# CODEJIN/multi_speaker_tts

Hardware: AMD Instinct MI355X
Metric: mel-frames/sec (train step) at batch 32x(128 tok,800 mel) (higher is better)
Workload: dtype f32

## Files before the change

include/mstts.h:

```cpp
#ifndef MSTTS_H_
#define MSTTS_H_
#include <stdint.h>
#ifdef __cplusplus
extern "C" {
#endif

typedef void* mstts_stream_t;

enum { MSTTS_OK = 0, MSTTS_ERR_SHAPE = -1, MSTTS_ERR_DTYPE = -2, MSTTS_ERR_ALIGN = -3, MSTTS_ERR_LAUNCH = -4 };
enum { MSTTS_ACT_NONE = 0, MSTTS_ACT_RELU = 1, MSTTS_ACT_TANH = 2, MSTTS_ACT_SIGMOID = 3 };

const char* mstts_last_error(void);
int mstts_abi_version(void);
int mstts_debug_park_cus(int32_t n_workgroups, int64_t microseconds, uint32_t* done_count, mstts_stream_t s);

typedef struct {
    const float* A; const float* B; float* C; const float* bias;
    int64_t M, N, K;
    int64_t lda, ldb, ldc;
    int32_t trans_a, trans_b;
    int32_t win_T, win_C, win_pad;
    int32_t act, accumulate, split_k;
    int64_t batch, stride_a, stride_b, stride_c;
    float alpha;
    int32_t win_dil;
} mstts_gemm_desc;
int mstts_gemm_f32(const mstts_gemm_desc* d, mstts_stream_t s);
int mstts_gemm_tail_split(int32_t on);
int mstts_gemm_split3(int32_t on);
int mstts_gemm_split_big(int32_t on);
int mstts_gemm_big_min_workgroups(int32_t f32_split, int32_t bf16);
int mstts_gemm_deterministic(int32_t on);
int mstts_gemm_bf16(const mstts_gemm_desc* d, mstts_stream_t s);
int mstts_gemm_bf16_autocut(int32_t on);
int mstts_gemm_bf16_big(int32_t on);

int mstts_philox_keep_mask(uint8_t* out, int64_t n, uint64_t seed, uint32_t stream_id, float keep_prob, mstts_stream_t s);
int mstts_philox_keep_mask_rows(uint8_t* out, int64_t outer, int64_t B, int64_t inner, uint64_t seed, uint32_t stream_id,
                                uint64_t sample0, float keep_prob, mstts_stream_t s);

int mstts_embedding_fwd(const int32_t* token, const float* table, float* out, int64_t n, int64_t vocab, int64_t width, mstts_stream_t s);
int mstts_embedding_bwd(const int32_t* token, const float* dout, float* dtable, int64_t n, int64_t vocab, int64_t width, mstts_stream_t s);

int mstts_bn_train_fwd(const float* x, const float* gamma, const float* beta, float* moving_mean, float* moving_var,
                       float* y, float* save_mean, float* save_rstd, const uint8_t* keep_mask, float keep_prob,
                       float momentum, float eps, int64_t rows, int64_t C, float* ws, mstts_stream_t s);
int mstts_bn_infer_fwd(const float* x, const float* gamma, const float* beta, const float* moving_mean,
                       const float* moving_var, float* y, float eps, int64_t rows, int64_t C, mstts_stream_t s);
int mstts_bn_train_bwd(const float* dy, const float* x, const float* gamma, const float* save_mean, const float* save_rstd,
                       const uint8_t* keep_mask, float keep_prob, int32_t act, float* dz, float* dgamma, float* dbeta,
                       float* dbias, int64_t rows, int64_t C, float* ws, mstts_stream_t s);

int mstts_dropout(const float* x, const uint8_t* keep_mask, float keep_prob, float* y, int64_t n, mstts_stream_t s);
int mstts_relu_dropout_bwd(const float* dy, const float* y_saved, const uint8_t* keep_mask, float keep_prob, float* dx, int64_t n, mstts_stream_t s);
int mstts_colsum(const float* x, int64_t rows, int64_t C, int64_t ld, float* out, int32_t accumulate, mstts_stream_t s);
// ... 399 lines not shown
```

multi_speaker_tts_amd/csrc/gemm.hip:

```cpp
#include "gemm_tile.h"
#include <type_traits>
#include <cmath>
#include <cstdlib>

namespace mstts {

constexpr int BK = 32;
constexpr int BN = 128;

struct GemmArgs : GemmTileArgs {
    int body, tail_s, tail_kps;
    int band;
};

template <int R, bool VEC>
struct LoaderKC {
    static constexpr int NV = R * BK / 4 / 256;
    float4 reg[NV];
    const float* ubase;
    unsigned voff[NV], rmask;
    int t_row[NV], tap, kc, ld_;
    __device__ __forceinline__ void prepare(const float* __restrict__ base, long ld, int row0, int k0, int rows,
                                            int wT, int wC, int wpad, int wdil) {
        const int k4 = threadIdx.x & 7, r = threadIdx.x >> 3;
        rmask = 0; ld_ = (int)ld;
#pragma unroll
        for (int i = 0; i < NV; ++i) {
            const int row = row0 + r + i * 32;
            if (row < rows) rmask |= 1u << i;
            voff[i] = (unsigned)((r + i * 32) * (int)ld) + (wT > 0 ? 0u : (unsigned)(k4 * 4));
            if (wT > 0) t_row[i] = row % wT;
        }
        if (wT > 0) {
            const int k = k0 + k4 * 4;
            tap = k / wC; kc = k - tap * wC;
// ... 223 lines not shown
#include "gemm_split.inc"

}

using namespace mstts;

static int g_tail_split = 1;
extern "C" int mstts_gemm_tail_split(int32_t on) { g_tail_split = on != 0; return MSTTS_OK; }
static int g_split3 = 1;
extern "C" int mstts_gemm_split3(int32_t on) { g_split3 = on != 0; return MSTTS_OK; }
static int g_split_big = 1;
extern "C" int mstts_gemm_split_big(int32_t on) { g_split_big = on != 0; return MSTTS_OK; }
static int g_split_big_min = 160;
namespace mstts { void gemm_bf16_set_big_min(int n); }
extern "C" int mstts_gemm_big_min_workgroups(int32_t f32_split, int32_t bf16) {
    if (f32_split > 0) g_split_big_min = f32_split;
    gemm_bf16_set_big_min(bf16);
    return MSTTS_OK;
}
static thread_local int t_deterministic = 0;
extern "C" int mstts_gemm_deterministic(int32_t on) { t_deterministic = on != 0; return MSTTS_OK; }
namespace mstts { int gemm_deterministic_now() { return t_deterministic; } }

extern "C" int mstts_gemm_f32(const mstts_gemm_desc* d, mstts_stream_t stream) {
    GemmArgs g;
    bool vec;
    const int rc = gemm_args_from(d, "gemm", BK, 1 << 24, &g, &vec);
    if (rc != MSTTS_OK || g.M == 0 || g.N == 0) return rc;
    const int batch = d->batch > 0 ? (int)d->batch : 1, split = g.split_k, kps = g.k_per_split;
    const bool skinny = d->M <= 32;
    int bm = skinny ? 32 : 128, tail_s = 1, tail_rem = 0;
    const bool split3 = g_split3 && !skinny && d->K >= 160 && (d->win_T <= 0 || (d->win_T >= BK && d->win_C >= BK)) && gemm_ready<GemmSplit>();
    if (!skinny) {
        const double t128 = (double)cdiv(d->M, 128) * cdiv(d->N, BN) * batch * split, t64 = (double)cdiv(d->M, 64) * cdiv(d->N, BN) * batch * split;
        const double e128 = t128 / (ceil(t128 / 256.0) * 256.0), e64 = t64 / (ceil(t64 / 256.0) * 256.0);
        if (e64 * 0.95 > e128 && !split3) bm = 64;
        if (g_tail_split && !t_deterministic && batch == 1 && split == 1 && (d->act == MSTTS_ACT_NONE || !d->accumulate)) {
            double best = (bm == 128 ? ceil(t128 / 256.0) : ceil(t64 / 256.0) * 0.54);
            const int ktiles = cdiv(d->K, BK);
            for (int cand = 128; cand >= (split3 ? 128 : 64); cand -= 64) {
                const long t = (long)cdiv(d->M, cand) * cdiv(d->N, BN);
                int rem = (int)(t % 256);
                if (d->act != MSTTS_ACT_NONE) rem = (int)(t - (t - rem) / cdiv(d->N, BN) * cdiv(d->N, BN));
                if (split3 && t <= 128) rem = (int)t;
                else if (t <= 256 || rem == 0 || rem > 128) continue;
                int s = 256 / rem;
                if (s > 16) s = 16;
                if (s > ktiles / 8) s = ktiles / 8;
                if (s < 2) continue;
                const double c = ((double)(t / 256) + 1.25 / s + 0.06) * (cand == 128 ? 1.0 : 0.54);
                if (c < best) { best = c; bm = cand; tail_s = s; tail_rem = rem; }
            }
        }
    }
    hipStream_t st = (hipStream_t)stream;
    const bool ta = d->trans_a != 0, tb = d->trans_b != 0, win = g.win_T > 0;
    {
        const long big_wgs = (long)cdiv(d->M, GSB_BM) * cdiv(d->N, GSB_BN) * batch * split;
        if (split3 && g_split_big && d->M >= 192 && d->N >= 192 && big_wgs >= g_split_big_min && d->lda < (1 << 22) && d->ldb < (1 << 22) &&
            (d->win_T <= 0 || (d->win_T >= GSB_BK && d->win_C >= GSB_BK)) && (d->act == MSTTS_ACT_NONE || split == 1) && gemm_ready<GemmSplitBig>()) {
            const int kpsb = gemm_k_per_split(g.K, split, GSB_BK);
            g.k_per_split = kpsb;
            g.body = 0; g.tail_s = 1; g.tail_kps = kpsb; g.band = 0;
            dim3 gridb(cdiv(d->M, GSB_BM) * cdiv(d->N, GSB_BN), 1, batch * split);
            gemm_launch<GemmSplitBig>(g, ta, tb, vec, win, gridb, st);
            MSTTS_CHECK_LAUNCH("gemm_f32 (split, 256 x 256 tile)");
            return MSTTS_OK;
        }
    }
    const int tiles = cdiv(d->M, bm) * cdiv(d->N, BN);
    g.body = tiles; g.tail_s = 1; g.tail_kps = kps;
    g.band = (split3 && tail_s == 1 && cdiv(d->N, BN) > 8) ? 8 : 0;
    if (tail_s > 1) {
        const int rem = tail_rem, tiles_n = cdiv(d->N, BN);
        g.body = tiles - rem; g.tail_s = tail_s;
        g.tail_kps = (cdiv(g.K, BK) + tail_s - 1) / tail_s * BK;
        if (!d->accumulate) {
            const long r0 = (long)(g.body / tiles_n) * bm;
            if (hipMemset2DAsync(d->C + r0 * d->ldc, (size_t)d->ldc * 4, 0, (size_t)d->N * 4, (size_t)(d->M - r0), st) != hipSuccess)
                MSTTS_REQUIRE(false, MSTTS_ERR_LAUNCH, "gemm: clearing the tail tiles failed");
        }
    }
    dim3 grid(g.body + (tiles - g.body) * g.tail_s, 1, batch * split);
    if (split3) gemm_launch<GemmSplit>(g, ta, tb, vec, win, grid, st);
    else if (skinny) gemm_launch<GemmF32<32>>(g, ta, tb, vec, win, grid, st);
    else if (bm == 64) gemm_launch<GemmF32<64>>(g, ta, tb, vec, win, grid, st);
    else gemm_launch<GemmF32<128>>(g, ta, tb, vec, win, grid, st);
    MSTTS_CHECK_LAUNCH("gemm_f32");
    if (tail_s > 1 && d->act != MSTTS_ACT_NONE) {
        const long r0 = (long)(g.body / cdiv(d->N, BN)) * bm;
        const long n = (d->M - r0) * d->N;
        hipLaunchKernelGGL(gemm_tail_act_kernel, dim3((unsigned)cdiv(n, 256)), dim3(256), 0, st, d->C + r0 * d->ldc, d->ldc, (int)d->N, n, d->act);
        MSTTS_CHECK_LAUNCH("gemm_f32 tail activation");
    }
    return MSTTS_OK;
}
```

multi_speaker_tts_amd/csrc/gemm_split.inc:

```

typedef __bf16 gs_bf16x8 __attribute__((ext_vector_type(8)));
typedef __bf16 gs_bf16x4 __attribute__((ext_vector_type(4)));
constexpr int GS_BM = 128, GS_LD = 40;
constexpr int GS_PLANE = 128 * GS_LD;

struct Split3 { gs_bf16x4 hi, mid, lo; };
__device__ __forceinline__ uint32_t gs_cvt_pk(float a, float b) {
    uint32_t r;
    asm("v_cvt_pk_bf16_f32 %0, %1, %2" : "=v"(r) : "v"(a), "v"(b));
    return r;
}
__device__ __forceinline__ float gs_sub(float a, uint32_t b_bits) {
    float r;
    asm("v_sub_f32 %0, %1, %2" : "=v"(r) : "v"(a), "v"(b_bits));
    return r;
}
__device__ __forceinline__ void gs_split2(float x0, float x1, uint32_t& hi, uint32_t& mid, uint32_t& lo) {
    hi = gs_cvt_pk(x0, x1);
    x0 = gs_sub(x0, hi << 16); x1 = gs_sub(x1, hi & 0xffff0000u);
    mid = gs_cvt_pk(x0, x1);
    x0 = gs_sub(x0, mid << 16); x1 = gs_sub(x1, mid & 0xffff0000u);
    lo = gs_cvt_pk(x0, x1);
}
__device__ __forceinline__ Split3 gs_split4(float a, float b, float c, float d) {
// ... 227 lines not shown
                acc[i][j] = __builtin_amdgcn_mfma_f32_32x32x16_bf16(f[i], fb[j][pb], acc[i][j], 0, 0, 0);
    };

    if (nt > 0) {
        load(kbeg);
        store(0);
        load(kbeg + GSB_BK);
        gemm_barrier();
        for (int t = 0; t < nt; ++t) {
            const __bf16* buf = gs_lds + (t & 1) * GSB_BUF;
            ldB(buf); ldA(fa0, buf, 0); ldA(fa1, buf, 1);
            mm(fa0, 0); mm(fa0, 1); mm(fa0, 2);
            ldA(fa0, buf, 2);
            store((t + 1) & 1);
            load(kbeg + (t + 2) * GSB_BK);
            mm(fa1, 0); mm(fa1, 1);
            mm(fa0, 0);
            gemm_barrier();
        }
    }
    gemm_store_tile<4, 2>(g, acc, C, m0 + wrow, n0 + wcol, lane, split == 0, g.split_k > 1);
}

struct GemmSplit {
    using Args = GemmArgs;
    static constexpr int THREADS = GS_THREADS;
    static constexpr size_t LDS_BYTES = GS_LDS_BYTES;
    template <bool TA, bool TB, bool VEC, bool WIN> static constexpr auto kernel() { return &gemm_split_kernel<TA, TB, VEC, WIN>; }
};
struct GemmSplitBig {
    using Args = GemmArgs;
    static constexpr int THREADS = GSB_THREADS;
    static constexpr size_t LDS_BYTES = GSB_LDS_BYTES;
    template <bool TA, bool TB, bool VEC, bool WIN> static constexpr auto kernel() { return &gemm_split_big_kernel<TA, TB, VEC, WIN>; }
};
```

multi_speaker_tts_amd/engine.py:

```python
from __future__ import annotations

import ctypes as C
import os
import warnings

import numpy as np
import torch

from . import lib
from .lib import ACT_NONE, ACT_RELU, ACT_TANH, gemm, ptr, call
from .masks import MaskSet, step_seed
from .params import CELL, ENC_CELL, LSA, LSA_VARS, VOC, Dims, ParamStore, bank_suffix
from .persist import PERSIST_COOLDOWN, PERSIST_STRIKES, CoolDown, Ticket, decoder_workgroups, lstm_bwd_workgroups, lstm_fwd_workgroups, near_xcd
from .training import (Engine, _split_k, _split_k_big, bn_train_fwd, conv_bn_bwd, conv_fwd, exponential_decay, lstm_layer_grads, lstm_seq_bwd,
                       lstm_seq_fwd)

MAX_PLANS = 64



def learning_rate(step):
    from . import Hyper_Parameters as hp
    return exponential_decay(hp.Train.Learning_Rate, step)


VOC_OVERLAP = os.environ.get("MSTTS_VOC_OVERLAP", "1") != "0"
POSTNET_WGRAD_OVERLAP = os.environ.get("MSTTS_POSTNET_WGRAD_OVERLAP", "1") != "0"
ENC_TAIL_OVERLAP = os.environ.get("MSTTS_ENC_TAIL_OVERLAP", "1") != "0"
ENC_OVERLAP = os.environ.get("MSTTS_ENC_OVERLAP", "1") != "0"


class _WS:
    """Attribute bag of device buffers for one (B, T_enc, L) shape: views into the engine's workspace arena."""


class _LateScalars:

# ... 110 lines not shown
        self.persist_selftest = 0
        self.persist_bwd_selftest = 0
        self.persist_stamps = None
        self.persist_bwd = self.persist and os.environ.get("MSTTS_PERSIST_BWD", "1") != "0" and bool(lb.mstts_persist_bwd_supported(1, H, M, d.att, 1, d.att_k))
        self.persist_bwd_fallbacks = 0
        self.speaker_ticket_redos = 0
        self.trace_events, self.bptt_end_event = False, None
        self.collective_redos = 0
        self.persist_bwd_stamps = None
        if self.persist:
            self.pk = [self._f(int(lb.mstts_persist_pack_floats(i))) for i in range(3)]
        self.persist_enc = os.environ.get("MSTTS_PERSIST_ENC", "1") != "0" and bool(lb.mstts_persist_lstm_supported(1, He))
        self.persist_enc_fallbacks = 0
        if self.persist_enc:
            n = int(lb.mstts_persist_lstm_pack_floats())
            self.enc_pk = {dr: (self._f(n), self._f(n)) for dr in ("fw", "bw")}
        if self.device.type == "cuda":
            self._side = torch.cuda.Stream(device=self.device)
            self._enc_stream = torch.cuda.Stream(device=self.device)
            self._voc_stream = self._enc_stream
        if self.persist_bwd:
            self.pkb = [self._f(int(lb.mstts_persist_bwd_pack_floats(i))) for i in range(3)]
        self.flip = {}
        self.big_tiles = os.environ.get("MSTTS_SPLIT_K_BIG", "1") != "0"
        self._derived_stale = True
        self.gemm_dtype = (gemm_dtype or "f32").lower()
        if self.gemm_dtype not in ("f32", "bf16"):
            raise ValueError("gemm_dtype must be 'f32' or 'bf16'")
        self.recurrent_dtype = (recurrent_dtype or "f32").lower()
        if self.recurrent_dtype not in ("f32", "bf16"):
            raise ValueError("recurrent_dtype must be 'f32' or 'bf16'")
        self.bf = None
        if self.recurrent_dtype == "bf16" and lb.mstts_cell_fwd_bf16_supported(H, M + H) and lb.mstts_cell_fwd_bf16_supported(H, 2 * H):
            self.w0p16 = torch.zeros((M + H) * 4 * H, dtype=torch.int16, device=self.device)
            self.w1p16 = torch.zeros(2 * H * 4 * H, dtype=torch.int16, device=self.device)
        if self.recurrent_dtype == "bf16":
            sp = (C.c_int32 * 6)()
            if not lib.load().mstts_decoder_bf16_splits(H, M, d.att, sp):
                raise ValueError("bf16 recurrent products need dec_lstm, mem and att widths that are multiples of 64")
            i16 = lambda n: torch.zeros(n, dtype=torch.int16, device=self.device)
            self.bf = {"splits": list(sp), "w0f_f": i16((M + H) * 4 * H), "w1_f": i16(2 * H * 4 * H), "wq_f": i16(H * d.att),
                       "w0f_b": i16((M + H) * 4 * H), "w1_b": i16(2 * H * 4 * H), "wq_b": i16(H * d.att)}

    def _gemm(self, *a, exact=False, **k):
        bf = self.gemm_dtype == "bf16" and not exact
        if self.deterministic and k.get("split_k", 1) > 1:
# ... 48 lines not shown
        k0, o0 = self.P(CELL % 0 + "kernel")
        call("mstts_fold_rows", ptr(k0, o0 + Pn * 4 * H), ptr(self.w0f), 2 * M + H, 4 * H, 0, M)
        self._fallback_packs_stale = True
        if not (self.persist and self.persist_bwd and self.persist_enc):
            self._ensure_fallback_packs()
        k1, o1 = self.P(CELL % 1 + "kernel"); wq_, oq_ = self.P(LSA + "query_layer/kernel")
        if self.persist_enc:
            cin_e, He = d.enc_conv_ch, d.enc_lstm
            for dr in ("fw", "bw"):
                ke, oke = self.P(ENC_CELL % dr + "kernel")
                call("mstts_persist_lstm_pack", ptr(ke, oke + cin_e * 4 * He), 4 * He, ptr(self.enc_pk[dr][0]), ptr(self.enc_pk[dr][1]))
        if self.persist:
            call("mstts_persist_pack", ptr(self.w0f), ptr(k1, o1), ptr(wq_, oq_), ptr(k0, o0), ptr(self.pk[0]), ptr(self.pk[1]), ptr(self.pk[2]))
        if self.persist_bwd:
            call("mstts_persist_bwd_pack", ptr(self.w0f), ptr(k1, o1), ptr(wq_, oq_), ptr(self.pkb[0]), ptr(self.pkb[1]), ptr(self.pkb[2]))
        wp, owp = self.P("decoder/decoder/linear_projection/dense/kernel")
        bp, obp = self.P("decoder/decoder/linear_projection/dense/bias")
        nm1 = d.n_mel + 1
        self.wp_pad.zero_()
        self.bp_pad.zero_()
        call("mstts_copy2d", ptr(wp, owp), nm1, ptr(self.wp_pad), self.proj_ld, H + M, nm1, 0)
        call("mstts_copy2d", ptr(bp, obp), nm1, ptr(self.bp_pad), self.proj_ld, 1, nm1, 0)
        lib.lsa_fold(self.P, self.loc_k, self.loc_b, self.loc_kt, d.att_k, d.att_ch, d.att)
        self._derived_stale = False

    def _pin(self, name, n):
        if name not in self._pinned:
            self._pinned[name] = torch.zeros(n, dtype=torch.int32).pin_memory()
        return self._pinned[name]

    def plan(self, B, Te, L):
        key = (B, Te, L)
        w = self._plans.get(key)
        if w is not None and w.arena_generation == self._arena.generation:
            self._plans[key] = self._plans.pop(key)
        else:
            cv = _Carver(self._arena, self._arena.buf is None)
            w, need = self._build_plan(B, Te, L, cv)
            if cv.count or cv.overflow:
                if self._arena.buf is None and self.arena_hint is not None:
                    hb, ht, hl = self.arena_hint
                    need = max(need, self._build_plan(max(B, hb), max(Te, ht), max(L, hl), _Carver(self._arena, True))[1])
                if self._arena.ensure(need):
                    self._plans.clear()
                    self._active_plan = None
                w = self._build_plan(B, Te, L, _Carver(self._arena, False))[0]
# ... 696 lines not shown
```

multi_speaker_tts_amd/lib.py:

```python
from __future__ import annotations

import ctypes as C
import os

import torch

from .params import LSA_VARS

_HERE = os.path.dirname(os.path.abspath(__file__))
LIB_PATH = os.path.join(_HERE, "libmstts_hip.so")

ACT_NONE, ACT_RELU, ACT_TANH, ACT_SIGMOID = 0, 1, 2, 3

vp, i64, i32, f32, u64, u32 = C.c_void_p, C.c_int64, C.c_int32, C.c_float, C.c_uint64, C.c_uint32


class GemmDesc(C.Structure):
    _fields_ = [("A", vp), ("B", vp), ("C", vp), ("bias", vp),
                ("M", i64), ("N", i64), ("K", i64), ("lda", i64), ("ldb", i64), ("ldc", i64),
                ("trans_a", i32), ("trans_b", i32), ("win_T", i32), ("win_C", i32), ("win_pad", i32),
                ("act", i32), ("accumulate", i32), ("split_k", i32),
                ("batch", i64), ("stride_a", i64), ("stride_b", i64), ("stride_c", i64), ("alpha", f32), ("win_dil", i32)]


class LstmPointFwd(C.Structure):
    _fields_ = [("B", i64), ("H", i64), ("gates_h", vp), ("gates_parts", i32), ("gates_pstride", i64), ("xw", vp), ("xw_sb", i64), ("xw_st", i64), ("bias", vp),
                ("c_prev", vp), ("h_prev", vp), ("h_prev_ld", i64), ("zc", vp), ("zh", vp), ("zoneout", f32),
                ("lengths", vp), ("step", i32), ("reverse", i32), ("residual", vp), ("res_sb", i64), ("res_st", i64),
                ("out", vp), ("out_sb", i64), ("out_st", i64), ("c_next", vp), ("h_next", vp), ("h_next_ld", i64),
                ("acts_out", vp), ("c_raw", vp)]


class LstmPointBwd(C.Structure):
    _fields_ = [("B", i64), ("H", i64), ("d_out", vp), ("dout_sb", i64), ("dout_st", i64), ("dout_parts", i32), ("dout_pstride", i64),
                ("d_out2", vp), ("dout2_parts", i32), ("dout2_pstride", i64),
                ("d_c_state", vp), ("d_h_state", vp), ("d_h_state2", vp), ("dhs2_ld", i64), ("dhs2_parts", i32), ("dhs2_pstride", i64),
                ("acts", vp), ("c_raw", vp), ("c_prev", vp), ("zc", vp), ("zh", vp), ("zoneout", f32),
                ("lengths", vp), ("step", i32), ("reverse", i32), ("dgates", vp), ("dgates_pos", vp),
                ("dgp_sb", i64), ("dgp_st", i64), ("d_c_prev", vp), ("d_h_prev", vp), ("dq", vp), ("wq_t", vp), ("A", i64), ("dq_bf16", i32)]


class CellPackedDst(C.Structure):
    _fields_ = [("base", vp), ("K", i64), ("col0", i64), ("bf16", i32)]


# ... 54 lines not shown
                ("xch", vp), ("ctrl", vp), ("stamps", vp), ("selftest_fail_step", i32), ("near_xcd", i32)]


class DecoderTrainBwd(C.Structure):
    _fields_ = [("fwd", C.POINTER(DecoderTrain)), ("d_pj", vp), ("dg0", vp), ("dg1", vp), ("dq_hist", vp),
                ("de_hist", vp), ("d_in0", vp), ("ws", vp)]


class DecoderInfer(C.Structure):
    _fields_ = [("B", i64), ("H", i64), ("P", i64), ("n_mel", i64), ("Smax", i64), ("lsa", LsaConst),
                ("pw0", vp), ("pb0", vp), ("pw1", vp), ("pb1", vp), ("pm0", vp), ("pm1", vp), ("prenet_keep", f32),
                ("wx0", vp), ("b0", vp), ("w0f", vp), ("w1", vp), ("b1", vp), ("wq", vp), ("wproj", vp), ("bproj", vp),
                ("zoneout", f32), ("in0", vp), ("in1", vp), ("pj", vp), ("c0", vp), ("c1", vp), ("cum", vp),
                ("pre_ws", vp), ("linear", vp), ("stop", vp), ("align_hist", vp), ("w0s", vp), ("wp_pad", vp), ("w0sp", vp), ("w1p", vp), ("act_p", vp), ("wp_own", vp), ("vp", vp)]


P = C.POINTER
SIGNATURES = {
    "mstts_last_error": (C.c_char_p, []),
    "mstts_abi_version": (i32, []),
    "mstts_debug_park_cus": (i32, [i32, i64, vp, vp]),
    "mstts_gemm_f32": (i32, [P(GemmDesc), vp]),
    "mstts_gemm_tail_split": (i32, [i32]),
    "mstts_gemm_split3": (i32, [i32]),
    "mstts_gemm_deterministic": (i32, [i32]),
    "mstts_gemm_split_big": (i32, [i32]),
    "mstts_gemm_big_min_workgroups": (i32, [i32, i32]),
    "mstts_gemm_bf16_autocut": (i32, [i32]),
    "mstts_persist_status": (i32, [vp, i32, vp, i32, vp, vp]),
    "mstts_gemm_bf16": (i32, [P(GemmDesc), vp]),
    "mstts_gemm_bf16_big": (i32, [i32]),
    "mstts_philox_keep_mask": (i32, [vp, i64, u64, u32, f32, vp]),
    "mstts_philox_keep_mask_rows": (i32, [vp, i64, i64, i64, u64, u32, u64, f32, vp]),
    "mstts_embedding_fwd": (i32, [vp, vp, vp, i64, i64, i64, vp]),
    "mstts_embedding_bwd": (i32, [vp, vp, vp, i64, i64, i64, vp]),
    "mstts_bn_train_fwd": (i32, [vp, vp, vp, vp, vp, vp, vp, vp, vp, f32, f32, f32, i64, i64, vp, vp]),
    "mstts_bn_infer_fwd": (i32, [vp, vp, vp, vp, vp, vp, f32, i64, i64, vp]),
    "mstts_bn_train_bwd": (i32, [vp, vp, vp, vp, vp, vp, f32, i32, vp, vp, vp, vp, i64, i64, vp, vp]),
    "mstts_dropout": (i32, [vp, vp, f32, vp, i64, vp]),
    "mstts_relu_dropout_bwd": (i32, [vp, vp, vp, f32, vp, i64, vp]),
    "mstts_colsum": (i32, [vp, i64, i64, i64, vp, i32, vp]),
    "mstts_add": (i32, [vp, vp, vp, i64, vp]),
    "mstts_fill": (i32, [vp, f32, i64, vp]),
    "mstts_copy2d": (i32, [vp, i64, vp, i64, i64, i64, i32, vp]),
    "mstts_maxpool2_same": (i32, [vp, vp, i64, i64, i64, vp]),
    "mstts_highway_combine": (i32, [vp, vp, vp, vp, i64, vp]),
# ... 165 lines not shown
        except RuntimeError as e:
            if "hipcc not found" in str(e) and os.path.exists(LIB_PATH) and not os.path.exists(LIB_PATH + ".hash"):
                import warnings
                warnings.warn("libmstts_hip.so could not be checked against its sources (hipcc not found); loading the existing library")
            else:
                raise
    lib = C.CDLL(LIB_PATH)
    for name, (res, args) in SIGNATURES.items():
        fn = getattr(lib, name)
        fn.restype = res
        fn.argtypes = args
    if lib.mstts_abi_version() != ABI_VERSION:
        raise MsttsError("libmstts_hip.so reports ABI version %d, this binding is written for %d: rebuild the library (python -m multi_speaker_tts_amd.build --force)"
                         % (lib.mstts_abi_version(), ABI_VERSION))
    env = os.environ.get
    if env("MSTTS_GEMM_SPLIT3", "1") == "0":
        lib.mstts_gemm_split3(0)
    if env("MSTTS_GEMM_SPLIT_BIG", "1") == "0":
        lib.mstts_gemm_split_big(0)
    if env("MSTTS_GEMM_BF16_BIG", "1") == "0":
        lib.mstts_gemm_bf16_big(0)
    if env("MSTTS_GEMM_BF16_AUTOCUT", "1") == "0":
        lib.mstts_gemm_bf16_autocut(0)
    if env("MSTTS_GEMM_SPLIT_BIG_MIN") or env("MSTTS_GEMM_BF16_BIG_MIN"):
        lib.mstts_gemm_big_min_workgroups(int(env("MSTTS_GEMM_SPLIT_BIG_MIN", "0")), int(env("MSTTS_GEMM_BF16_BIG_MIN", "0")))
    _lib = lib
    return lib


class deterministic_gemm:
    _depth = __import__("threading").local()

    def __enter__(self):
        n = getattr(self._depth, "n", 0)
        if n == 0:
            load().mstts_gemm_deterministic(1)
        self._depth.n = n + 1
        return self

    def __exit__(self, *exc):
        self._depth.n -= 1
        if self._depth.n == 0:
            load().mstts_gemm_deterministic(0)
        return False

    def __call__(self, fn):
# ... 23 lines not shown

def call(name, *args):
    lib = load()
    rc = getattr(lib, name)(*args, stream())
    if rc != 0:
        raise MsttsError("%s failed (%d): %s" % (name, rc, lib.mstts_last_error().decode()))


def lsa_fold(P, loc_k, loc_b, loc_kt, KS, CH, A):
    src = [ptr(*P(name)) for _, name in LSA_VARS[:3]]
    call("mstts_lsa_fold_location", *src, ptr(loc_k), ptr(loc_b), KS, CH, A)
    if loc_kt is not None:
        call("mstts_lsa_filter_by_unit", ptr(loc_k), ptr(loc_kt), KS, A)


def lsa_fill(ls, P, B, T, A, M, KS, CH, keys, values, lengths, loc_k, loc_b, loc_kt):
    ls.B, ls.T, ls.A, ls.M, ls.KS, ls.CH = B, T, A, M, KS, CH
    ls.keys, ls.values, ls.lengths = ptr(keys), ptr(values), ptr(lengths)
    for field, name in LSA_VARS:
        setattr(ls, field, ptr(*P(name)))
    ls.loc_k, ls.loc_b, ls.loc_kt = ptr(loc_k), ptr(loc_b), ptr(loc_kt)


def gemm(A, B, Cm, M, N, K, lda, ldb, ldc, bias=None, trans_a=False, trans_b=False, act=ACT_NONE, accumulate=False,
         split_k=1, win=None, batch=1, strides=(0, 0, 0), alpha=1.0, a_off=0, b_off=0, c_off=0, bias_off=0, bf16=False):
    d = GemmDesc()
    d.A, d.B, d.C, d.bias = ptr(A, a_off), ptr(B, b_off), ptr(Cm, c_off), ptr(bias, bias_off)
    d.M, d.N, d.K, d.lda, d.ldb, d.ldc = M, N, K, lda, ldb, ldc
    d.trans_a, d.trans_b = int(trans_a), int(trans_b)
    if win is not None:
        d.win_T, d.win_C, d.win_pad = win[:3]
        d.win_dil = win[3] if len(win) > 3 else 1
    d.act, d.accumulate, d.split_k = act, int(accumulate), split_k
    d.batch, d.stride_a, d.stride_b, d.stride_c = batch, strides[0], strides[1], strides[2]
    d.alpha = alpha
    call("mstts_gemm_bf16" if bf16 else "mstts_gemm_f32", C.byref(d))
```

multi_speaker_tts_amd/training.py:

```python
from __future__ import annotations

import math
import os
import time

import numpy as np
import torch

from . import Hyper_Parameters as hp
from . import lib
from .lib import call, ptr

BN_MOM, BN_EPS = 0.99, 1e-3

MAX_PLANS = 3


def _split_k(M, N, K, n_cu=256, max_split=16):
    tiles = math.ceil(M / 128) * math.ceil(N / 128)
    if K >= 16384:
        ktiles, best, best_cost = K / 32.0, 1, None
        if tiles * max_split < n_cu:
            max_split = min(64, max(max_split, n_cu // tiles))
        for sk in range(1, max_split + 1):
# ... 77 lines not shown


def lstm_seq_fwd(B, T, H, xw, wh, lengths, reverse, zoneout, zc, zh, out, out_sb, out_st, c_hist, h_hist, acts, c_raw, gates_ws, residual=None):
    return lib.LstmSeqFwd(B=B, T=T, H=H, xw=ptr(xw), wh=ptr(*wh), wh_ld=4 * H, lengths=ptr(lengths), reverse=reverse, zoneout=zoneout,
                          zc=ptr(zc), zh=ptr(zh), residual=ptr(residual), out=ptr(*out), out_sb=out_sb, out_st=out_st,
                          c_hist=ptr(c_hist), h_hist=ptr(h_hist), acts=ptr(acts), c_raw=ptr(c_raw), gates_ws=ptr(gates_ws))


def lstm_seq_bwd(B, T, H, wh, lengths, reverse, zoneout, zc, zh, d_out, dout_sb, dout_st, c_hist, acts, c_raw, dgates_step, dgates_pos, ws):
    return lib.LstmSeqBwd(B=B, T=T, H=H, wh=ptr(*wh), wh_ld=4 * H, lengths=ptr(lengths), reverse=reverse, zoneout=zoneout,
                          zc=ptr(zc), zh=ptr(zh), d_out=ptr(*d_out), dout_sb=dout_sb, dout_st=dout_st, c_hist=ptr(c_hist), acts=ptr(acts),
                          c_raw=ptr(c_raw), dgates_step=ptr(dgates_step), dgates_pos=ptr(dgates_pos), ws=ptr(ws))


def lstm_layer_grads(eng, gemm, cell, x, h, dgp, dgs, dx, rows, cin, H, dx_accumulate=False):
    k, ok = eng.P(cell + "kernel")
    gk, ogk = eng.G(cell + "kernel"); gb, ogb = eng.G(cell + "bias")
    gemm(x, dgp, gk, cin, 4 * H, rows, cin, 4 * H, 4 * H, trans_a=True, split_k=max(2, _split_k(cin, 4 * H, rows)), c_off=ogk)
    gemm(h, dgs, gk, H, 4 * H, rows, H, 4 * H, 4 * H, trans_a=True, split_k=max(2, _split_k(H, 4 * H, rows)), c_off=ogk + cin * 4 * H)
    call("mstts_colsum", ptr(dgs), rows, 4 * H, 4 * H, ptr(gb, ogb), 1)
    gemm(dgp, k, dx, rows, cin, 4 * H, 4 * H, 4 * H, cin, trans_b=True, accumulate=dx_accumulate, b_off=ok)


def conv_fwd(eng, gemm, x, rows, T, cin, cout, K, conv, out, act):
    k, ok = eng.P(conv + "/kernel"); b, ob = eng.P(conv + "/bias")
    gemm(x, k, out, rows, cout, K * cin, cin, cout, cout, bias=b, act=act, win=(T, cin, (K - 1) // 2), b_off=ok, bias_off=ob)


def bn_train_fwd(eng, bn, a, y, mean, rstd, mask, keep, rows, C, ws):
    g, og = eng.P(bn + "gamma"); b, ob = eng.P(bn + "beta")
    mm, omm = eng.P(bn + "moving_mean"); mv, omv = eng.P(bn + "moving_variance")
    call("mstts_bn_train_fwd", ptr(a), ptr(g, og), ptr(b, ob), ptr(mm, omm), ptr(mv, omv), ptr(y), ptr(mean), ptr(rstd),
         ptr(mask), float(keep), BN_MOM, BN_EPS, rows, C, ptr(ws))


def conv_bn_bwd(eng, gemm, conv, bn, dy, x_in, a, mean, rstd, mask, keep, act, rows, T, cin, cout, K, dz, dx, ws, dx_accumulate=False,
                wgrad_stream=None):
    g, og = eng.P(bn + "gamma")
    gg, ogg = eng.G(bn + "gamma"); gb, ogb = eng.G(bn + "beta"); gbias, ogbias = eng.G(conv + "/bias")
    call("mstts_bn_train_bwd", ptr(dy), ptr(a), ptr(g, og), ptr(mean), ptr(rstd), ptr(mask), float(keep), act, ptr(dz),
         ptr(gg, ogg), ptr(gb, ogb), ptr(gbias, ogbias), rows, cout, ptr(ws))
    gk, ogk = eng.G(conv + "/kernel")
    pad = (K - 1) // 2
    wgrad = lambda: gemm(x_in, dz, gk, K * cin, cout, rows, cin, cout, cout, trans_a=True, win=(T, cin, pad),
                         split_k=max(2, _split_k(K * cin, cout, rows)), c_off=ogk)
    if wgrad_stream is None:
        wgrad()
    else:
        ev = torch.cuda.Event()
        ev.record()
        with torch.cuda.stream(wgrad_stream):
            wgrad_stream.wait_event(ev)
            wgrad()
    if dx is not None:
        k, ok = eng.P(conv + "/kernel")
        key = (conv, K, cin, cout)
        if key not in eng.flip:
            eng.flip[key] = eng._f(K, cout, cin)
        wt = eng.flip[key]
        call("mstts_conv_kernel_flip", ptr(k, ok), ptr(wt), K, cin, cout)
        gemm(dz, wt, dx, rows, cin, K * cout, cout, cin, cin, win=(T, cout, K - 1 - pad), accumulate=dx_accumulate)


class DropIn:
    HP = FILE = SCOPE = None
    COLUMNS = ()

    def _file(self):
        return os.path.join(getattr(hp, self.HP).Checkpoint_Path.replace("\\", "/"), self.FILE)

    def _slots(self):
        return {"__adam_m__": self.params.adam_m, "__adam_v__": self.params.adam_v}

    def Restore(self):
        f = self._file()
        if not os.path.exists(f):
            print("There is no checkpoint.")
            return
        state = torch.load(f, map_location="cpu")
        self.params.load({k: v for k, v in state.items() if k.startswith(self.SCOPE)})
        if "__adam_m__" in state:
            for k, t in self._slots().items():
                t.copy_(state[k])
        self.engine.global_step = int(state.get("__global_step__", 0))
# ... 22 lines not shown
```

Baseline: 643,500.

## Add conv-form split GEMM with prepacked bf16-split weights and sliding A slab

Adds a specialized split-bf16 GEMM kernel for windowed convolution GEMMs. It loads one A row slab per channel block and reuses it across all taps by shifting row offsets, rather than re-gathering im2col tiles for each tap. Weights are prepacked once per parameter version into a three-plane bf16 image laid out per tile, which removes the per-call split and the kernel flip in the backward pass. In exchange it adds pack buffers, a refresh launch whenever parameters change, and edge-masking logic for padded taps.

After: 647,800, median of 6. No clear change (+0.7%).

```diff
diff --git a/include/mstts.h b/include/mstts.h
--- a/include/mstts.h
+++ b/include/mstts.h
@@ -31,6 +31,16 @@
 int mstts_gemm_split_big(int32_t on);
 int mstts_gemm_big_min_workgroups(int32_t f32_split, int32_t bf16);
 int mstts_gemm_deterministic(int32_t on);
+typedef struct {
+    const float* w; void* pack;
+    int64_t taps, cin, cout;
+    int32_t flip, reserved;
+} mstts_conv_pack_seg;
+int64_t mstts_conv_pack_bytes(int64_t taps, int64_t win_c, int64_t n);
+int mstts_conv_pack_build(const mstts_conv_pack_seg* segs, int32_t n, mstts_stream_t s);
+int mstts_gemm_f32_packed(const mstts_gemm_desc* d, const void* pack, mstts_stream_t s);
+int mstts_gemm_conv_form_takes(const mstts_gemm_desc* d);
+int mstts_gemm_conv_form(int32_t on);
 int mstts_gemm_bf16(const mstts_gemm_desc* d, mstts_stream_t s);
 int mstts_gemm_bf16_autocut(int32_t on);
 int mstts_gemm_bf16_big(int32_t on);
diff --git a/multi_speaker_tts_amd/csrc/gemm.hip b/multi_speaker_tts_amd/csrc/gemm.hip
--- a/multi_speaker_tts_amd/csrc/gemm.hip
+++ b/multi_speaker_tts_amd/csrc/gemm.hip
@@ -11,6 +11,7 @@
 struct GemmArgs : GemmTileArgs {
     int body, tail_s, tail_kps;
     int band;
+    const void* bpack;
 };
 
 template <int R, bool VEC>
@@ -280,12 +281,38 @@
 extern "C" int mstts_gemm_deterministic(int32_t on) { t_deterministic = on != 0; return MSTTS_OK; }
 namespace mstts { int gemm_deterministic_now() { return t_deterministic; } }
 
-extern "C" int mstts_gemm_f32(const mstts_gemm_desc* d, mstts_stream_t stream) {
+static int g_conv_form = 1;
+extern "C" int mstts_gemm_conv_form(int32_t on) { g_conv_form = on != 0; return MSTTS_OK; }
+
+static bool gemm_big_shape(const mstts_gemm_desc* d, int batch, int split) {
+    const long big_wgs = (long)cdiv(d->M, GSB_BM) * cdiv(d->N, GSB_BN) * batch * split;
+    return g_split_big && d->M >= 192 && d->N >= 192 && big_wgs >= g_split_big_min && d->lda < (1 << 22) && d->ldb < (1 << 22) &&
+           (d->act == MSTTS_ACT_NONE || split == 1);
+}
+static bool gemm_takes_conv_form(const mstts_gemm_desc* d, bool vec, int batch, int split) {
+    if (!g_conv_form || !g_split3 || d->win_T <= 0 || d->trans_a || d->trans_b || batch != 1 || !vec || d->win_dil > 1) return false;
+    if (d->win_C % GSB_BK != 0 || d->K % d->win_C != 0) return false;
+    const long taps = d->K / d->win_C;
+    if (taps < GSC_MIN_TAPS || taps > GSC_MAX_TAPS || d->win_pad < 0 || d->win_pad >= taps) return false;
+    return gemm_big_shape(d, batch, split) && gemm_ready<GemmSplitConv>();
+}
+
+static int gemm_f32_run(const mstts_gemm_desc* d, const void* pack, mstts_stream_t stream) {
     GemmArgs g;
     bool vec;
     const int rc = gemm_args_from(d, "gemm", BK, 1 << 24, &g, &vec);
     if (rc != MSTTS_OK || g.M == 0 || g.N == 0) return rc;
+    g.bpack = nullptr;
     const int batch = d->batch > 0 ? (int)d->batch : 1, split = g.split_k, kps = g.k_per_split;
+    if (pack != nullptr && gemm_takes_conv_form(d, vec, batch, split)) {
+        g.bpack = pack;
+        g.k_per_split = cdiv(g.win_C / GSB_BK, split);
+        g.body = 0; g.tail_s = 1; g.tail_kps = 0; g.band = 0;
+        dim3 gridc(cdiv(d->M, GSB_BM) * cdiv(d->N, GSB_BN), 1, split);
+        gemm_launch<GemmSplitConv>(g, false, false, true, true, gridc, (hipStream_t)stream);
+        MSTTS_CHECK_LAUNCH("gemm_f32 (split, conv form)");
+        return MSTTS_OK;
+    }
     const bool skinny = d->M <= 32;
     int bm = skinny ? 32 : 128, tail_s = 1, tail_rem = 0;
     const bool split3 = g_split3 && !skinny && d->K >= 160 && (d->win_T <= 0 || (d->win_T >= BK && d->win_C >= BK)) && gemm_ready<GemmSplit>();
@@ -314,9 +341,7 @@
     hipStream_t st = (hipStream_t)stream;
     const bool ta = d->trans_a != 0, tb = d->trans_b != 0, win = g.win_T > 0;
     {
-        const long big_wgs = (long)cdiv(d->M, GSB_BM) * cdiv(d->N, GSB_BN) * batch * split;
-        if (split3 && g_split_big && d->M >= 192 && d->N >= 192 && big_wgs >= g_split_big_min && d->lda < (1 << 22) && d->ldb < (1 << 22) &&
-            (d->win_T <= 0 || (d->win_T >= GSB_BK && d->win_C >= GSB_BK)) && (d->act == MSTTS_ACT_NONE || split == 1) && gemm_ready<GemmSplitBig>()) {
+        if (split3 && gemm_big_shape(d, batch, split) && (d->win_T <= 0 || (d->win_T >= GSB_BK && d->win_C >= GSB_BK)) && gemm_ready<GemmSplitBig>()) {
             const int kpsb = gemm_k_per_split(g.K, split, GSB_BK);
             g.k_per_split = kpsb;
             g.body = 0; g.tail_s = 1; g.tail_kps = kpsb; g.band = 0;
@@ -353,3 +378,37 @@
     }
     return MSTTS_OK;
 }
+
+extern "C" int mstts_gemm_f32(const mstts_gemm_desc* d, mstts_stream_t stream) { return gemm_f32_run(d, nullptr, stream); }
+extern "C" int mstts_gemm_f32_packed(const mstts_gemm_desc* d, const void* pack, mstts_stream_t stream) { return gemm_f32_run(d, pack, stream); }
+extern "C" int mstts_gemm_conv_form_takes(const mstts_gemm_desc* d) {
+    GemmArgs g;
+    bool vec;
+    if (gemm_args_from(d, "gemm", BK, 1 << 24, &g, &vec) != MSTTS_OK || g.M == 0 || g.N == 0) return 0;
+    return gemm_takes_conv_form(d, vec, d->batch > 0 ? (int)d->batch : 1, g.split_k) ? 1 : 0;
+}
+
+extern "C" int64_t mstts_conv_pack_bytes(int64_t taps, int64_t C, int64_t N) {
+    if (taps < GSC_MIN_TAPS || taps > GSC_MAX_TAPS || C <= 0 || C % GSB_BK != 0 || N <= 0) return 0;
+    return (int64_t)cdiv(N, GSB_BN) * (C / GSB_BK) * taps * GSC_IMG * (int64_t)sizeof(__bf16);
+}
+extern "C" int mstts_conv_pack_build(const mstts_conv_pack_seg* segs, int32_t n, mstts_stream_t stream) {
+    MSTTS_REQUIRE(n >= 0 && (n == 0 || segs != nullptr), MSTTS_ERR_SHAPE, "conv_pack_build: bad segment table");
+    for (int s0 = 0; s0 < n; s0 += CONV_PACK_MAX_SEGS) {
+        ConvPackArgs a;
+        a.n = n - s0 < CONV_PACK_MAX_SEGS ? n - s0 : CONV_PACK_MAX_SEGS;
+        long chunks = 0;
+        for (int i = 0; i < a.n; ++i) {
+            const mstts_conv_pack_seg& q = segs[s0 + i];
+            const int64_t C = q.flip ? q.cout : q.cin, N = q.flip ? q.cin : q.cout;
+            MSTTS_REQUIRE(q.w && q.pack && aligned16(q.pack) && mstts_conv_pack_bytes(q.taps, C, N) > 0 && q.cin * q.cout * q.taps < (1LL << 31), MSTTS_ERR_SHAPE,
+                          "conv_pack_build: segment %d needs 3..8 taps, a window width that is a multiple of 16 and a 16-byte aligned pack", s0 + i);
+            chunks += mstts_conv_pack_bytes(q.taps, C, N) / (3 * 16);
+            a.seg[i] = ConvPackSeg{q.w, (__bf16*)q.pack, (int)q.taps, (int)C, (int)N, q.flip != 0, chunks};
+        }
+        if (chunks == 0) continue;
+        hipLaunchKernelGGL(conv_pack_kernel, dim3((unsigned)cdiv(chunks, 256)), dim3(256), 0, (hipStream_t)stream, a);
+        MSTTS_CHECK_LAUNCH("conv_pack_build");
+    }
+    return MSTTS_OK;
+}
diff --git a/multi_speaker_tts_amd/csrc/gemm_split.inc b/multi_speaker_tts_amd/csrc/gemm_split.inc
--- a/multi_speaker_tts_amd/csrc/gemm_split.inc
+++ b/multi_speaker_tts_amd/csrc/gemm_split.inc
@@ -273,11 +273,193 @@
     gemm_store_tile<4, 2>(g, acc, C, m0 + wrow, n0 + wcol, lane, split == 0, g.split_k > 1);
 }
 
+constexpr int GSC_SLAB_ROWS = 264;
+constexpr int GSC_SLAB_PLANE = GSC_SLAB_ROWS * GSB_LD;
+constexpr int GSC_SLAB = 3 * GSC_SLAB_PLANE;
+constexpr int GSC_BBUF = 3 * GSB_PLANE;
+constexpr size_t GSC_LDS_BYTES = (size_t)(2 * GSC_SLAB + 2 * GSC_BBUF) * sizeof(__bf16);
+constexpr int GSC_IMG = 3 * GSB_BN * GSB_BK;
+constexpr int GSC_MIN_TAPS = 3, GSC_MAX_TAPS = 8;
+
+typedef uint32_t gsc_u32x4 __attribute__((ext_vector_type(4)));
+typedef const gsc_u32x4 __attribute__((address_space(1)))* gsc_gptr4;
+
+__global__ __launch_bounds__(GSB_THREADS) void gemm_split_conv_kernel(GemmArgs g) {
+    extern __shared__ __attribute__((aligned(16))) __bf16 gs_lds[];
+    __bf16* const slabs = gs_lds;
+    __bf16* const bbufs = gs_lds + 2 * GSC_SLAB;
+    const int tiles_n = (g.N + GSB_BN - 1) / GSB_BN;
+    const int tile = gemm_xcd_tile(blockIdx.x, gridDim.x);
+    const int tile_m = tile / tiles_n, tile_n = tile % tiles_n;
+    const int split = blockIdx.z;
+    const int m0 = tile_m * GSB_BM, n0 = tile_n * GSB_BN;
+    const int wC = g.win_C, taps = g.K / wC, pad = g.win_pad, ncb = wC >> 4;
+    const int cb_beg = split * g.k_per_split, cb_end = min(ncb, cb_beg + g.k_per_split);
+    const int nt = cb_end > cb_beg ? (cb_end - cb_beg) * taps : 0;
+    const int tid = threadIdx.x, lane = tid & 63, wave = __builtin_amdgcn_readfirstlane(tid >> 6);
+    const int wrow = (wave >> 2) * 128, wcol = (wave & 3) * 64;
+    const int l31 = lane & 31, kg = lane >> 5;
+
+    const int k4 = tid & 3, r = tid >> 2;
+    const float* const abase = g.A + ((long)m0 - pad) * wC + (long)cb_beg * GSB_BK;
+    const int emax = (255 + taps - 1 - r) >> 7;
+    const int gm = m0 - pad + r;
+    auto lda = [&](int e, int cb) {
+        const int row = gm + e * 128;
+        const bool ok = row >= 0 && row < g.M && cb < cb_end;
+        return gemm_ld4(ok ? abase + (cb - cb_beg) * GSB_BK + (unsigned)((r + e * 128) * wC + k4 * 4) : gemm_zero16);
+    };
+    auto sta = [&](__bf16* slab, int e, const float4& v) { SplitPlanes<GSC_SLAB_PLANE>::put(slab + (r + e * 128) * GSB_LD + k4 * 4, v.x, v.y, v.z, v.w); };
+    const int bn = ((tid >> 4) << 3) + (tid & 7), bh = (tid >> 3) & 1;
+    const __bf16* const bimg = (const __bf16*)g.bpack + ((long)tile_n * ncb + cb_beg) * taps * GSC_IMG + (bn * 2 + bh) * 8;
+    const int bdst = bn * GSB_LD + bh * 8;
+    gsc_u32x4 rb[3];
+    auto ldb = [&](int t) {
+#pragma unroll
+        for (int p = 0; p < 3; ++p)
+            rb[p] = *(gsc_gptr4)(t < nt ? (const void*)(bimg + (long)t * GSC_IMG + p * (GSB_BN * GSB_BK)) : (const void*)gemm_zero16);
+    };
+    auto stb = [&](__bf16* bb) {
+#pragma unroll
+        for (int p = 0; p < 3; ++p) *reinterpret_cast<gsc_u32x4*>(bb + p * GSB_PLANE + bdst) = rb[p];
+    };
+
+    unsigned zm = 0;
+#pragma unroll
+    for (int i = 0; i < 4; ++i) {
+        const int tr = (m0 + wrow + i * 32 + l31) % g.win_T;
+        for (int j = 0; j < taps; ++j) {
+            const int ts = tr + j - pad;
+            if (ts < 0 || ts >= g.win_T) zm |= 1u << (8 * i + j);
+        }
+    }
+    const bool edge = __builtin_amdgcn_readfirstlane((int)(__ballot(zm != 0) != 0ull)) != 0;
+
+    f32x16 acc[4][2];
+#pragma unroll
+    for (int i = 0; i < 4; ++i)
+#pragma unroll
+        for (int j = 0; j < 2; ++j)
+#pragma unroll
+            for (int q = 0; q < 16; ++q) acc[i][j][q] = 0.f;
+
+    const int aoff = (wrow + l31) * GSB_LD + kg * 8, boff = (wcol + l31) * GSB_LD + kg * 8;
+    gs_bf16x8 fb[2][3], fa0[4], fa1[4];
+    constexpr int zoff = (GSC_SLAB_ROWS - 1) * GSB_LD;
+    int ao[4];
+    auto tapA = [&](int j) {
+#pragma unroll
+        for (int i = 0; i < 4; ++i) ao[i] = aoff + (i * 32 + j) * GSB_LD;
+        if (edge) {
+#pragma unroll
+            for (int i = 0; i < 4; ++i) ao[i] = ((zm >> (8 * i + j)) & 1u) ? zoff + kg * 8 : ao[i];
+        }
+    };
+    auto ldA = [&](gs_bf16x8 (&f)[4], const __bf16* slab, int p) {
+#pragma unroll
+        for (int i = 0; i < 4; ++i) f[i] = *reinterpret_cast<const gs_bf16x8*>(slab + ao[i] + p * GSC_SLAB_PLANE);
+    };
+    auto ldB = [&](const __bf16* bb) {
+#pragma unroll
+        for (int p = 0; p < 3; ++p)
+#pragma unroll
+            for (int j = 0; j < 2; ++j) fb[j][p] = *reinterpret_cast<const gs_bf16x8*>(bb + boff + p * GSB_PLANE + j * 32 * GSB_LD);
+    };
+    auto mm = [&](const gs_bf16x8 (&f)[4], int pb) {
+#pragma unroll
+        for (int i = 0; i < 4; ++i)
+#pragma unroll
+            for (int j = 0; j < 2; ++j)
+                acc[i][j] = __builtin_amdgcn_mfma_f32_32x32x16_bf16(f[i], fb[j][pb], acc[i][j], 0, 0, 0);
+    };
+
+    if (nt > 0) {
+        if (tid < 72) reinterpret_cast<uint32_t*>(slabs + (tid / 12) * GSC_SLAB_PLANE + zoff)[tid % 12] = 0u;
+        float4 ra;
+#pragma unroll
+        for (int e = 0; e < 3; ++e) { ra = lda(min(e, emax), cb_beg); sta(slabs, min(e, emax), ra); }
+        ldb(0); stb(bbufs);
+        ldb(1);
+        ra = lda(0, cb_beg + 1);
+        gemm_barrier();
+        int j = 0, cb = cb_beg, par = 0;
+        for (int t = 0; t < nt; ++t) {
+            const __bf16* slab = slabs + par * GSC_SLAB;
+            __bf16* next = slabs + (par ^ 1) * GSC_SLAB;
+            const __bf16* bb = bbufs + (t & 1) * GSC_BBUF;
+            tapA(j);
+            ldB(bb); ldA(fa0, slab, 0); ldA(fa1, slab, 1);
+            mm(fa0, 0); mm(fa0, 1); mm(fa0, 2);
+            ldA(fa0, slab, 2);
+            stb(bbufs + ((t + 1) & 1) * GSC_BBUF);
+            sta(next, min(j, emax), ra);
+            const bool last = j == taps - 1;
+            ra = lda(last ? 0 : min(j + 1, emax), last ? cb + 2 : cb + 1);
+            ldb(t + 2);
+            mm(fa1, 0); mm(fa1, 1);
+            mm(fa0, 0);
+            gemm_barrier();
+            j = last ? 0 : j + 1; cb += last ? 1 : 0; par ^= last ? 1 : 0;
+        }
+    }
+    gemm_store_tile<4, 2>(g, acc, g.C, m0 + wrow, n0 + wcol, lane, split == 0, g.split_k > 1);
+}
+
+constexpr int CONV_PACK_MAX_SEGS = 16;
+struct ConvPackSeg { const float* w; __bf16* out; int taps, C, N, flip; long chunk_end; };
+struct ConvPackArgs { ConvPackSeg seg[CONV_PACK_MAX_SEGS]; int n; };
+
+__global__ __launch_bounds__(256) void conv_pack_kernel(ConvPackArgs a) {
+    long c = (long)blockIdx.x * 256 + threadIdx.x;
+    int s = 0;
+    while (s < a.n && c >= a.seg[s].chunk_end) ++s;
+    if (s >= a.n) return;
+    if (s > 0) c -= a.seg[s - 1].chunk_end;
+    const float* __restrict__ w = a.seg[s].w;
+    const int taps = a.seg[s].taps, C = a.seg[s].C, N = a.seg[s].N, ncb = C >> 4;
+    const int half = (int)(c & 1), nn = (int)((c >> 1) & (GSB_BN - 1));
+    long img = c >> 9;
+    const int tap = (int)(img % taps); img /= taps;
+    const int cb = (int)(img % ncb), tile_n = (int)(img / ncb);
+    const int n = tile_n * GSB_BN + nn, ch = cb * GSB_BK + half * 8;
+    float x[8];
+#pragma unroll
+    for (int i = 0; i < 8; ++i) x[i] = 0.f;
+    if (n < N) {
+        if (a.seg[s].flip) {
+            const float* p = w + ((long)(taps - 1 - tap) * N + n) * C + ch;
+#pragma unroll
+            for (int i = 0; i < 8; ++i) x[i] = p[i];
+        } else {
+            const float* p = w + ((long)tap * C + ch) * N + n;
+#pragma unroll
+            for (int i = 0; i < 8; ++i) x[i] = p[(long)i * N];
+        }
+    }
+    gsc_u32x4 hi, mid, lo;
+#pragma unroll
+    for (int i = 0; i < 4; ++i) {
+        uint32_t h, m, l;
+        gs_split2(x[2 * i], x[2 * i + 1], h, m, l);
+        hi[i] = h; mid[i] = m; lo[i] = l;
+    }
+    __bf16* o = a.seg[s].out + (c >> 9) * GSC_IMG + (long)(nn * 2 + half) * 8;
+    *reinterpret_cast<gsc_u32x4*>(o) = hi;
+    *reinterpret_cast<gsc_u32x4*>(o + GSB_BN * GSB_BK) = mid;
+    *reinterpret_cast<gsc_u32x4*>(o + 2 * GSB_BN * GSB_BK) = lo;
+}
+
 struct GemmSplit {
     using Args = GemmArgs;
     static constexpr int THREADS = GS_THREADS;
     static constexpr size_t LDS_BYTES = GS_LDS_BYTES;
     template <bool TA, bool TB, bool VEC, bool WIN> static constexpr auto kernel() { return &gemm_split_kernel<TA, TB, VEC, WIN>; }
+};
+struct GemmSplitConv {
+    using Args = GemmArgs;
+    static constexpr int THREADS = GSB_THREADS;
+    static constexpr size_t LDS_BYTES = GSC_LDS_BYTES;
+    template <bool TA, bool TB, bool VEC, bool WIN> static constexpr auto kernel() { return &gemm_split_conv_kernel; }
 };
 struct GemmSplitBig {
     using Args = GemmArgs;
diff --git a/multi_speaker_tts_amd/engine.py b/multi_speaker_tts_amd/engine.py
--- a/multi_speaker_tts_amd/engine.py
+++ b/multi_speaker_tts_amd/engine.py
@@ -12,7 +12,7 @@
 from .masks import MaskSet, step_seed
 from .params import CELL, ENC_CELL, LSA, LSA_VARS, VOC, Dims, ParamStore, bank_suffix
 from .persist import PERSIST_COOLDOWN, PERSIST_STRIKES, CoolDown, Ticket, decoder_workgroups, lstm_bwd_workgroups, lstm_fwd_workgroups, near_xcd
-from .training import (Engine, _split_k, _split_k_big, bn_train_fwd, conv_bn_bwd, conv_fwd, exponential_decay, lstm_layer_grads, lstm_seq_bwd,
+from .training import (Engine, _split_k, _split_k_big, bn_train_fwd, conv_bn_bwd, conv_fwd, conv_packs_refresh, exponential_decay, lstm_layer_grads, lstm_seq_bwd,
                        lstm_seq_fwd)
 
 MAX_PLANS = 64
@@ -169,6 +169,7 @@
         if self.persist_bwd:
             self.pkb = [self._f(int(lb.mstts_persist_bwd_pack_floats(i))) for i in range(3)]
         self.flip = {}
+        self.conv_packs, self._conv_packs_version = {}, -1
         self.big_tiles = os.environ.get("MSTTS_SPLIT_K_BIG", "1") != "0"
         self._derived_stale = True
         self.gemm_dtype = (gemm_dtype or "f32").lower()
@@ -263,6 +264,7 @@
         call("mstts_copy2d", ptr(wp, owp), nm1, ptr(self.wp_pad), self.proj_ld, H + M, nm1, 0)
         call("mstts_copy2d", ptr(bp, obp), nm1, ptr(self.bp_pad), self.proj_ld, 1, nm1, 0)
         lib.lsa_fold(self.P, self.loc_k, self.loc_b, self.loc_kt, d.att_k, d.att_ch, d.att)
+        conv_packs_refresh(self)
         self._derived_stale = False
 
     def _pin(self, name, n):
diff --git a/multi_speaker_tts_amd/lib.py b/multi_speaker_tts_amd/lib.py
--- a/multi_speaker_tts_amd/lib.py
+++ b/multi_speaker_tts_amd/lib.py
@@ -21,6 +21,10 @@
                 ("trans_a", i32), ("trans_b", i32), ("win_T", i32), ("win_C", i32), ("win_pad", i32),
                 ("act", i32), ("accumulate", i32), ("split_k", i32),
                 ("batch", i64), ("stride_a", i64), ("stride_b", i64), ("stride_c", i64), ("alpha", f32), ("win_dil", i32)]
+
+
+class ConvPackSeg(C.Structure):
+    _fields_ = [("w", vp), ("pack", vp), ("taps", i64), ("cin", i64), ("cout", i64), ("flip", i32), ("reserved", i32)]
 
 
 class LstmPointFwd(C.Structure):
@@ -121,6 +125,11 @@
     "mstts_debug_park_cus": (i32, [i32, i64, vp, vp]),
     "mstts_gemm_f32": (i32, [P(GemmDesc), vp]),
     "mstts_gemm_tail_split": (i32, [i32]),
+    "mstts_gemm_f32_packed": (i32, [P(GemmDesc), vp, vp]),
+    "mstts_gemm_conv_form_takes": (i32, [P(GemmDesc)]),
+    "mstts_gemm_conv_form": (i32, [i32]),
+    "mstts_conv_pack_bytes": (i64, [i64, i64, i64]),
+    "mstts_conv_pack_build": (i32, [P(ConvPackSeg), i32, vp]),
     "mstts_gemm_split3": (i32, [i32]),
     "mstts_gemm_deterministic": (i32, [i32]),
     "mstts_gemm_split_big": (i32, [i32]),
@@ -332,6 +341,8 @@
         lib.mstts_gemm_bf16_big(0)
     if env("MSTTS_GEMM_BF16_AUTOCUT", "1") == "0":
         lib.mstts_gemm_bf16_autocut(0)
+    if env("MSTTS_GEMM_CONV_FORM", "1") == "0":
+        lib.mstts_gemm_conv_form(0)
     if env("MSTTS_GEMM_SPLIT_BIG_MIN") or env("MSTTS_GEMM_BF16_BIG_MIN"):
         lib.mstts_gemm_big_min_workgroups(int(env("MSTTS_GEMM_SPLIT_BIG_MIN", "0")), int(env("MSTTS_GEMM_BF16_BIG_MIN", "0")))
     _lib = lib
@@ -401,8 +412,8 @@
     ls.loc_k, ls.loc_b, ls.loc_kt = ptr(loc_k), ptr(loc_b), ptr(loc_kt)
 
 
-def gemm(A, B, Cm, M, N, K, lda, ldb, ldc, bias=None, trans_a=False, trans_b=False, act=ACT_NONE, accumulate=False,
-         split_k=1, win=None, batch=1, strides=(0, 0, 0), alpha=1.0, a_off=0, b_off=0, c_off=0, bias_off=0, bf16=False):
+def _gemm_desc(A, B, Cm, M, N, K, lda, ldb, ldc, bias=None, trans_a=False, trans_b=False, act=ACT_NONE, accumulate=False,
+               split_k=1, win=None, batch=1, strides=(0, 0, 0), alpha=1.0, a_off=0, b_off=0, c_off=0, bias_off=0):
     d = GemmDesc()
     d.A, d.B, d.C, d.bias = ptr(A, a_off), ptr(B, b_off), ptr(Cm, c_off), ptr(bias, bias_off)
     d.M, d.N, d.K, d.lda, d.ldb, d.ldc = M, N, K, lda, ldb, ldc
@@ -413,4 +424,32 @@
     d.act, d.accumulate, d.split_k = act, int(accumulate), split_k
     d.batch, d.stride_a, d.stride_b, d.stride_c = batch, strides[0], strides[1], strides[2]
     d.alpha = alpha
-    call("mstts_gemm_bf16" if bf16 else "mstts_gemm_f32", C.byref(d))
+    return d
+
+
+def gemm(A, B, Cm, M, N, K, lda, ldb, ldc, bias=None, trans_a=False, trans_b=False, act=ACT_NONE, accumulate=False,
+         split_k=1, win=None, batch=1, strides=(0, 0, 0), alpha=1.0, a_off=0, b_off=0, c_off=0, bias_off=0, bf16=False, pack=None):
+    d = _gemm_desc(A, B, Cm, M, N, K, lda, ldb, ldc, bias, trans_a, trans_b, act, accumulate, split_k, win, batch, strides, alpha,
+                   a_off, b_off, c_off, bias_off)
+    if pack is not None and not bf16:
+        call("mstts_gemm_f32_packed", C.byref(d), ptr(pack))
+    else:
+        call("mstts_gemm_bf16" if bf16 else "mstts_gemm_f32", C.byref(d))
+
+
+def gemm_takes_conv_form(*a, **k):
+    return bool(load().mstts_gemm_conv_form_takes(C.byref(_gemm_desc(*a, **k))))
+
+
+def conv_pack_alloc(taps, win_c, n, device):
+    nbytes = int(load().mstts_conv_pack_bytes(taps, win_c, n))
+    return torch.empty(nbytes // 2, dtype=torch.int16, device=device) if nbytes else None
+
+
+def conv_packs_build(segs):
+    if not segs:
+        return
+    table = (ConvPackSeg * len(segs))()
+    for e, (w, off, pack, taps, cin, cout, flip) in zip(table, segs):
+        e.w, e.pack, e.taps, e.cin, e.cout, e.flip = ptr(w, off), ptr(pack), taps, cin, cout, int(flip)
+    call("mstts_conv_pack_build", table, len(segs))
diff --git a/multi_speaker_tts_amd/training.py b/multi_speaker_tts_amd/training.py
--- a/multi_speaker_tts_amd/training.py
+++ b/multi_speaker_tts_amd/training.py
@@ -123,9 +123,36 @@
     gemm(dgp, k, dx, rows, cin, 4 * H, 4 * H, 4 * H, cin, trans_b=True, accumulate=dx_accumulate, b_off=ok)
 
 
+def conv_packs_refresh(eng):
+    lib.conv_packs_build([seg for _, seg in eng.conv_packs.values()])
+    eng._conv_packs_version = eng.params.version
+
+
+def _conv_pack(eng, conv, K, cin, cout, flip, gemm_args, gemm_kw):
+    packs = getattr(eng, "conv_packs", None)
+    if packs is None or getattr(eng, "gemm_dtype", "f32") == "bf16":
+        return None
+    if not lib.gemm_takes_conv_form(*gemm_args, **gemm_kw):
+        return None
+    key = (conv, flip)
+    if key not in packs:
+        k, ok = eng.P(conv + "/kernel")
+        pk = lib.conv_pack_alloc(K, cout if flip else cin, cin if flip else cout, k.device)
+        packs[key] = (pk, (k, ok, pk, K, cin, cout, flip))
+        lib.conv_packs_build([packs[key][1]])
+    elif eng._conv_packs_version != eng.params.version:
+        conv_packs_refresh(eng)
+    return packs[key][0]
+
+
 def conv_fwd(eng, gemm, x, rows, T, cin, cout, K, conv, out, act):
     k, ok = eng.P(conv + "/kernel"); b, ob = eng.P(conv + "/bias")
-    gemm(x, k, out, rows, cout, K * cin, cin, cout, cout, bias=b, act=act, win=(T, cin, (K - 1) // 2), b_off=ok, bias_off=ob)
+    a = (x, k, out, rows, cout, K * cin, cin, cout, cout)
+    kw = dict(bias=b, act=act, win=(T, cin, (K - 1) // 2), b_off=ok, bias_off=ob)
+    pk = _conv_pack(eng, conv, K, cin, cout, False, a, kw)
+    if pk is not None:
+        kw["pack"] = pk
+    gemm(*a, **kw)
 
 
 def bn_train_fwd(eng, bn, a, y, mean, rstd, mask, keep, rows, C, ws):
@@ -159,8 +186,14 @@
         if key not in eng.flip:
             eng.flip[key] = eng._f(K, cout, cin)
         wt = eng.flip[key]
-        call("mstts_conv_kernel_flip", ptr(k, ok), ptr(wt), K, cin, cout)
-        gemm(dz, wt, dx, rows, cin, K * cout, cout, cin, cin, win=(T, cout, K - 1 - pad), accumulate=dx_accumulate)
+        a = (dz, wt, dx, rows, cin, K * cout, cout, cin, cin)
+        kw = dict(win=(T, cout, K - 1 - pad), accumulate=dx_accumulate)
+        pk = _conv_pack(eng, conv, K, cin, cout, True, a, kw)
+        if pk is not None:
+            kw["pack"] = pk
+        else:
+            call("mstts_conv_kernel_flip", ptr(k, ok), ptr(wt), K, cin, cout)
+        gemm(*a, **kw)
 
 
 class DropIn:
```
